# evanwporter/SparseCholesky

Measured on AMD Instinct MI355X. Metric: numeric-factorization fp64 GFLOP/s (F=sum colcount^2), higher is better.
Workload: dtype f64

## Files before the change

sparsecholesky_amd/csrc/kernels.hip:

```cpp
#include <hip/hip_runtime.h>

#include <cstdint>
#include <type_traits>

#include "kernels.hpp"

namespace sc {

typedef double double4_t __attribute__((ext_vector_type(4)));

__device__ __forceinline__ void report_fail(int32_t* info, const int32_t* post, int32_t col_internal) {
    atomicMin(info, (post ? post[col_internal] : col_internal) + 1);
}

__device__ __forceinline__ int bnd_at(const int32_t* b, int k, int mbc) {
    const int klo = b[0], khi = b[1];
    return k <= klo ? b[2] : (k >= khi ? mbc : b[2 + k - klo]);
}

__device__ __forceinline__ int lower_bound_i32(const int32_t* a, int n, int v) {
    int lo = 0, hi = n;
    while (lo < hi) {
        int mid = (lo + hi) >> 1;
        if (a[mid] < v)
// ... 839 lines not shown
            const double l = (ok && i > j) ? rec[j * 64 + i] / sqrt(d) : 0.0;
            lv[i] = l;
            wave_lds_sync();
            for (int k = j + 1; k < n; ++k)
                if (i >= k) rec[k * 64 + i] -= l * lv[k];
        }
    }
    if (i == 0) {
        if (T.host_info) {
            const int32_t st = fail < n ? nat + 1 : 0x7f7f7f7f;
            P.info[0] = st;
            __hip_atomic_store(T.host_info, st, __ATOMIC_RELEASE, __HIP_MEMORY_SCOPE_SYSTEM);
        } else if (fail < n) {
            atomicMin(P.info, nat + 1);
        }
    }
}

hipError_t launch_tiny_dense(const DevPlan& P, const TinyPlan& T, int n, const double* Ax, hipStream_t st) {
    if (n <= 0) return hipSuccess;
    if (n > TINY_DENSE_N || T.na != tiny_dense_np(n) * 64) return hipErrorInvalidValue;
    if ((int64_t)T.nax * 8 >= BUF_DEAD || (int64_t)T.npan * 8 >= BUF_DEAD) return hipErrorInvalidValue;
    if (n <= 16)
        hipLaunchKernelGGL(tiny_dense_kernel<16>, dim3(1), dim3(64), 0, st, P, T, n, Ax);
    else if (n <= 32)
        hipLaunchKernelGGL(tiny_dense_kernel<32>, dim3(1), dim3(64), 0, st, P, T, n, Ax);
    else if (n <= 48)
        hipLaunchKernelGGL(tiny_dense_kernel<48>, dim3(1), dim3(64), 0, st, P, T, n, Ax);
    else
        hipLaunchKernelGGL(tiny_dense_kernel<64>, dim3(1), dim3(64), 0, st, P, T, n, Ax);
    return hipGetLastError();
}

__global__ __launch_bounds__(256) void chain_init_kernel(DevPlan P, ChainPlan C, int first,
                                                          const double* __restrict__ Ax) {
    extern __shared__ double F[];
    const ChainDesc d = C.desc[first + blockIdx.x];
    small_assemble(P, d.s, d.c0, d.w, d.m, Ax, F, d.sp);
    const int tot = (d.m * (d.m + 1)) >> 1;
    double* out = C.init + d.init_off;
    for (int idx = threadIdx.x; idx < tot; idx += 256) out[idx] = F[idx];
}

#ifndef SC_CHAIN_DB
#define SC_CHAIN_DB 1
#endif
constexpr int CHAIN_IMG = (128 * 129 / 2 + CHAIN_NT - 1) / CHAIN_NT;
__global__ __launch_bounds__(CHAIN_NT) void front_chain_kernel(DevPlan P, ChainPlan C, int first, int count, int fsz) {
    extern __shared__ double F[];
    __shared__ __attribute__((aligned(16))) double colbuf[2 * 4 * COLB];
    __shared__ ChainDesc ds[CHAIN_MAXF];
    const int tid = threadIdx.x;
    for (int i = tid; i < count; i += CHAIN_NT) ds[i] = C.desc[first + i];
    lds_barrier();
    double img[CHAIN_IMG];
    int nbi, nbj;
    uint32_t nrr, nrc;
    auto prefetch = [&](int f) {
        const ChainDesc& d = ds[f];
        const int tot = (d.m * (d.m + 1)) >> 1;
        const double* src = C.init + d.init_off;
#pragma unroll
        for (int q = 0; q < CHAIN_IMG; ++q) {
            const int idx = tid + CHAIN_NT * q;
            img[q] = idx < tot ? src[idx] : 0.0;
        }
        const int T = (d.m + 3) >> 2;
        nbi = nbj = -1;
        if (tid < T * (T + 1) / 2) tile_map(tid, T, (d.w + 3) >> 2, nbi, nbj);
        nrr = nbi >= 0 ? C.relp[d.relp_off + nbi] : 0u;
        nrc = nbi >= 0 ? C.relp[d.relp_off + nbj] : 0u;
    };
    auto Fb = [&](int f) { return SC_CHAIN_DB ? F + (f & 1) * fsz : F; };
    auto put = [&](int f) {
        const int tot = (ds[f].m * (ds[f].m + 1)) >> 1;
        double* Fd = Fb(f);
#pragma unroll
        for (int q = 0; q < CHAIN_IMG; ++q) {
            const int idx = tid + CHAIN_NT * q;
            if (idx < tot) Fd[idx] = img[q];
        }
    };
    int cbi, cbj;
    uint32_t crr, crc;
    auto take = [&]() {
        cbi = nbi;
        cbj = nbj;
        crr = nrr;
        crc = nrc;
    };
    prefetch(0);
    put(0);
    take();
    if (count > 1) prefetch(1);
    lds_barrier();
    for (int i = 0; i < count; ++i) {
        uint64_t* stamp = C.stamps ? C.stamps + 8 * (first + i) : nullptr;
        if (stamp && tid == 0) stamp[0] = __builtin_amdgcn_s_memtime();
        const ChainDesc d = ds[i];
        const int m = d.m, w = d.w;
        SmallRegs<1> R;
        R.bi[0] = cbi;
        R.bj[0] = cbj;
        const uint32_t rr = crr, rc = crc;
        small_load<1>(R, Fb(i), m);
        if (!SC_CHAIN_DB) lds_barrier();
        if (stamp && tid == 0) stamp[1] = __builtin_amdgcn_s_memtime();
        const bool has_parent = i + 1 < count;
        if (has_parent) {
            put(i + 1);
            take();
            if (i + 2 < count) prefetch(i + 2);
        }
        if (stamp && tid == 0) stamp[2] = __builtin_amdgcn_s_memtime();
        small_steps<1>(R, colbuf, w, P.info, P.post, d.c0);
        if (w == 0) lds_barrier();
        if (stamp && tid == 0) stamp[3] = __builtin_amdgcn_s_memtime();
        small_store_panel<1>(R, P.panel_pool + d.panel_off, m, w);
        if (m > w && R.bi[0] >= 0 && 4 * R.bi[0] + 3 >= w) {
            if (!has_parent) {
                small_store_cb<1>(R, P.cb_pool + d.cb_off, m, w);
            } else {
                const int mp = ds[i + 1].m;
                double* Fp = Fb(i + 1);
#pragma unroll
                for (int r = 0; r < 4; ++r)
#pragma unroll
                    for (int c = 0; c < 4; ++c) {
                        const int ii = 4 * R.bi[0] + r, jj = 4 * R.bj[0] + c;
                        const int pr = (rr >> (8 * r)) & 255, pc = (rc >> (8 * c)) & 255;
                        if (jj >= w && ii >= jj && ii < m) Fp[pk_col(mp, pc) + pr - pc] += R.v[0][r * 4 + c];
                    }
            }
        }
        lds_barrier();
        if (stamp && tid == 0) stamp[4] = __builtin_amdgcn_s_memtime();
    }
}

#include "panel_gen.inc"

__global__ __launch_bounds__(256) void potrf_tiles_kernel(DevPlan P, const int2* __restrict__ tasks) {
    __shared__ __attribute__((aligned(16))) double colbuf[2 * 4 * COLB];
    const int2 t = tasks[blockIdx.x];
    const int s = t.x, k0 = t.y;
    const int c0 = P.sn_start[s];
    const int w = P.sn_start[s + 1] - c0;
    const int m = P.sn_m[s];
    const int nb = min(PNB, w - k0);
    double* blk = P.panel_pool + P.panel_off[s] + (int64_t)k0 * m + k0;
    SmallRegs<1> R;
    small_tiles<1>(R, nb, nb);
#pragma unroll
    for (int r = 0; r < 4; ++r)
#pragma unroll
        for (int c = 0; c < 4; ++c) {
            const int i = 4 * R.bi[0] + r, j = 4 * R.bj[0] + c;
            R.v[0][r * 4 + c] = (R.bi[0] >= 0 && i < nb && i >= j) ? blk[(int64_t)j * m + i] : 0.0;
        }
    if (SC_POTRF_FAST)
        small_steps1_fast(R, colbuf, nb, P.info, P.post, c0 + k0);
    else
        small_steps<1>(R, colbuf, nb, P.info, P.post, c0 + k0);
    if (R.bi[0] < 0) return;
#pragma unroll
    for (int r = 0; r < 4; ++r)
#pragma unroll
        for (int c = 0; c < 4; ++c) {
            const int i = 4 * R.bi[0] + r, j = 4 * R.bj[0] + c;
            if (i < nb && i >= j) blk[(int64_t)j * m + i] = R.v[0][r * 4 + c];
        }
}

__device__ __forceinline__ void trsm_partial(double* pan, int m, int k0, int nb, int r0, int nrows, double* Lc,
                                             double* invd) {
    constexpr int LD = PNB + 2;
    const int tid = threadIdx.x;
    const double* blk = pan + (int64_t)k0 * m + k0;
    for (int idx = tid; idx < PNB * PNB; idx += TRSM_ROWS) {
        const int q = idx % PNB, j = idx / PNB;
        const double v = (q < nb && j < nb && j <= q) ? blk[(int64_t)j * m + q] : 0.0;
        Lc[j * LD + q] = v;
        if (q == j) invd[j] = (j < nb) ? 1.0 / v : 0.0;
    }
    __syncthreads();
    const int row = r0 + tid;
    const bool live = row < m && tid < nrows;
    double* xs = pan + (int64_t)k0 * m + (live ? row : r0);
    double r[PNB];
#pragma unroll
    for (int c = 0; c < PNB; ++c) r[c] = (live && c < nb) ? xs[(int64_t)c * m] : 0.0;
    trsm_steps<0>(r, Lc, invd, nb);
    if (live) {
#pragma unroll
        for (int c = 0; c < PNB; ++c)
            if (c < nb) xs[(int64_t)c * m] = r[c];
    }
}

__global__ __launch_bounds__(TRSM_ROWS) void trsm_partial_kernel(DevPlan P, const TrsmTask* __restrict__ tasks) {
    __shared__ double Lc[PNB * (PNB + 2)];
    __shared__ double invd[PNB];
    const TrsmTask t = tasks[blockIdx.x];
    const int s = t.s, k0 = t.k0, r0 = t.r0;
    const int c0 = P.sn_start[s];
    const int w = P.sn_start[s + 1] - c0;
    const int m = P.sn_m[s];
    trsm_partial(P.panel_pool + P.panel_off[s], m, k0, min(PNB, w - k0), r0, min(TRSM_ROWS, t.r1 - r0), Lc, invd);
}

template <int PRE>
__global__ __launch_bounds__(TRSM_ROWS) void trsm_panel_g_kernel(DevPlan P, const TrsmTask* __restrict__ tasks,
                                                                 int32_t* __restrict__ arrive) {
    static_assert(TRSM_ROWS == 256, "the fused POTRF maps 4 x 4 tiles onto 256 threads");
    __shared__ double2 S[TRSM64_STREAM / 2];
    __shared__ __attribute__((aligned(16))) double colbuf[2 * 4 * COLB];
    __shared__ int s_last;
    const TrsmTask t = tasks[blockIdx.x];
    const int s = t.s, k0 = t.k0, r0 = t.r0, r1 = t.r1;
    const int tid = threadIdx.x;
    const int c0 = P.sn_start[s];
    const int w = P.sn_start[s + 1] - c0;
    const int m = P.sn_m[s];
    const int nb = min(PNB, w - k0);
    double* pan = P.panel_pool + P.panel_off[s];
    if (nb < PNB) return;
    double* blk = pan + (int64_t)k0 * m + k0;
    double* Sd = reinterpret_cast<double*>(S);
    SmallRegs<1> R;
    small_tiles<1>(R, PNB, PNB);
#pragma unroll
    for (int r = 0; r < 4; ++r)
#pragma unroll
        for (int c = 0; c < 4; ++c) {
            const int i = 4 * R.bi[0] + r, j = 4 * R.bj[0] + c;
            R.v[0][r * 4 + c] = (R.bi[0] >= 0 && i >= j) ? blk[(int64_t)j * m + i] : 0.0;
        }
    if constexpr (PRE == 2) {
        if (R.bi[0] >= 0) {
#pragma unroll
            for (int r = 0; r < 4; ++r)
#pragma unroll
                for (int c = 0; c < 4; ++c) {
                    const int i = 4 * R.bi[0] + r, j = 4 * R.bj[0] + c;
                    if (i >= j) Sd[PNB * j - j * (j - 1) / 2 + (i - j)] = (i == j) ? 1.0 / R.v[0][r * 4 + c] : R.v[0][r * 4 + c];
                }
        }
        const int row = r0 + tid;
        const __amdgpu_buffer_rsrc_t rs = buf_rsrc(pan + (int64_t)k0 * m, (uint32_t)m * PNB * 8u);
        const int voff = row < r1 ? row * 8 : BUF_DEAD;
        double r[PNB];
#pragma unroll
        for (int c = 0; c < PNB; ++c) r[c] = buf_ld(rs, voff, c * m * 8);
        __syncthreads();
        trsm64_full(r, S);
#pragma unroll
        for (int c = 0; c < PNB; ++c) buf_st(r[c], rs, voff, c * m * 8);
        return;
    }
    if (SC_POTRF_FAST)
        small_steps1_fast(R, colbuf, PNB, P.info, P.post, c0 + k0);
    else
        small_steps<1>(R, colbuf, PNB, P.info, P.post, c0 + k0);
    if (R.bi[0] >= 0) {
#pragma unroll
        for (int r = 0; r < 4; ++r)
#pragma unroll
            for (int c = 0; c < 4; ++c) {
                const int i = 4 * R.bi[0] + r, j = 4 * R.bj[0] + c;
                if (i >= j) Sd[PNB * j - j * (j - 1) / 2 + (i - j)] = (i == j) ? 1.0 / R.v[0][r * 4 + c] : R.v[0][r * 4 + c];
            }
    }
    const int row = r0 + tid;
    const __amdgpu_buffer_rsrc_t rs = buf_rsrc(pan + (int64_t)k0 * m, (uint32_t)m * PNB * 8u);
    const int voff = row < r1 ? row * 8 : BUF_DEAD;
    double r[PNB];
#pragma unroll
    for (int c = 0; c < PNB; ++c) r[c] = buf_ld(rs, voff, c * m * 8);
    __syncthreads();
    if (tid == 0) {
        const int k1 = k0 + PNB;
        const int nwg = (max(r1, k1 + 1) - k1 + TRSM_ROWS - 1) / TRSM_ROWS;
        const int old = __hip_atomic_fetch_add(arrive + (t.ctr - 1), 1, __ATOMIC_RELAXED, __HIP_MEMORY_SCOPE_AGENT);
        s_last = old == nwg - 1;
        if (old == nwg - 1) __hip_atomic_store(arrive + (t.ctr - 1), 0, __ATOMIC_RELAXED, __HIP_MEMORY_SCOPE_AGENT);
    }
    __syncthreads();
    if (s_last && R.bi[0] >= 0) {
#pragma unroll
        for (int rr = 0; rr < 4; ++rr)
#pragma unroll
            for (int c = 0; c < 4; ++c) {
                const int i = 4 * R.bi[0] + rr, j = 4 * R.bj[0] + c;
                if (i >= j) blk[(int64_t)j * m + i] = R.v[0][rr * 4 + c];
            }
    }
    trsm64_full(r, S);
#pragma unroll
    for (int c = 0; c < PNB; ++c) buf_st(r[c], rs, voff, c * m * 8);
}

#ifndef SC_PROBE_NOGATHER
#define SC_PROBE_NOGATHER 0
#endif
#ifndef SC_PROBE_NOK
#define SC_PROBE_NOK 0
#endif
template <int BT, int WM, int WN, int BK = 16, int GR = 64>
__device__ __forceinline__ void syrk_gather_epilogue(const GemmTask& T, const int64_t* __restrict__ gblk,
                                                     const GSeg* __restrict__ gseg, int row0, int col0,
                                                     double4_t (&acc)[BT / WM / 16][BT / WN / 16], double* smem) {
    constexpr int NW = WM * WN, NT = 64 * NW;
    constexpr int RTM = BT / WM / 16, RTN = BT / WN / 16;
    constexpr int GLD = GR + 1;
    constexpr int GQ = BT == 64 ? (GR == 32 ? 8 : 64 / NW) : SC_GATHER_Q;
    constexpr int SB = BT == 64 ? 4 : 1;
    constexpr int OPS = 2 * 2 * BK * (BT + 16);
    static_assert(BT * GLD <= OPS, "gather chunk fits the operand LDS");
    const int tid = threadIdx.x, lane = tid & 63, wid = tid >> 6;
    const int wr = wid / WN, wc = wid % WN;
    const int w = T.gw;
    const int mb = T.M;
    const int nb = (mb + 63) >> 6;
    const int64_t* __restrict__ blk = gblk + T.gb;
    const GSeg* __restrict__ seg = gseg;
    double* G = smem;
    double* __restrict__ C = T.C;
    const int64_t ldc = T.ldc;
    const __amdgpu_buffer_rsrc_t rc = buf_rsrc(C + (int64_t)col0 * ldc, (uint32_t)(min(BT, T.N - col0) * ldc * 8));
#pragma unroll 1
    for (int h = 0; h < BT / GR; ++h) {
        const int r0 = row0 + h * GR;
        const int rb = r0 >> 6;
        if (h) __syncthreads();
        for (int e = tid; e < BT * GLD; e += NT) G[e] = 0.0;
        __syncthreads();
        const int cb1 = min(min(nb, rb + 1), (col0 + BT) >> 6);
        for (int cbk = col0 >> 6; !SC_PROBE_NOGATHER && r0 < mb && cbk < cb1; ++cbk) {
            const int64_t bi = (int64_t)rb * (rb + 1) / 2 + cbk;
            const int64_t p0 = blk[bi], p1 = blk[bi + 1];
            for (int64_t pb = p0; pb < p1; pb += SB) {
                int prw[SB], pcl[SB];
#pragma unroll
                for (int q = 0; q < SB; ++q) {
                    prw[q] = -1;
                    pcl[q] = -1;
                    if (pb + q < p1) {
                        const GSeg& g = seg[pb + q];
                        const int ic = g.ilo + lane, jl = g.jlo + lane;
                        if (ic < g.ihi) prw[q] = g.rel[ic] - w - r0;
                        if (jl < g.jhi) pcl[q] = g.rel[jl] - w - col0;
                    }
                }
#pragma unroll
                for (int q = 0; q < SB; ++q) {
                    if (pb + q >= p1) break;
                    const GSeg& g = seg[pb + q];
                    const int ic = g.ilo + lane;
                    const int prow = prw[q] < GR ? prw[q] : -1;
                    const int mbc = g.mbc;
                    const double* __restrict__ cb = g.cb;
                    uint64_t mask = __ballot(pcl[q] >= 0 && pcl[q] % NW == wid);
                    while (mask) {
                        int jc[GQ], pc[GQ];
#pragma unroll
                        for (int u = 0; u < GQ; ++u) {
                            const int b = mask ? __builtin_ctzll(mask) : -1;
                            jc[u] = b < 0 ? -1 : g.jlo + b;
                            pc[u] = b < 0 ? 0 : __builtin_amdgcn_readlane(pcl[q], b);
                            mask &= mask - 1;
                        }
                        double v[GQ];
                        bool ok[GQ];
#pragma unroll
                        for (int u = 0; u < GQ; ++u) {
                            ok[u] = jc[u] >= 0 && prow >= 0 && ic >= jc[u];
                            const __amdgpu_buffer_rsrc_t rs = buf_rsrc(cb + (int64_t)max(jc[u], 0) * mbc, (uint32_t)mbc * 8u);
                            v[u] = buf_ld(rs, ok[u] ? ic * 8 : BUF_DEAD, 0);
                        }
#pragma unroll
                        for (int u = 0; u < GQ; ++u)
                            if (ok[u]) G[pc[u] * GLD + prow] += v[u];
                    }
                }
            }
        }
        __syncthreads();
        static_assert(GR % (BT / WM) == 0, "a wave's rows lie in one chunk");
        if ((wr * (BT / WM)) / GR == h) {
#pragma unroll
            for (int a = 0; a < RTM; ++a)
#pragma unroll
                for (int b = 0; b < RTN; ++b)
#pragma unroll
                    for (int r = 0; r < 4; ++r) {
                        const int lr = wr * (BT / WM) + a * 16 + MFMA_F64_ROW(lane, r);
                        const int lc = wc * (BT / WN) + b * 16 + (lane & 15);
                        G[lc * GLD + (lr - h * GR)] -= acc[a][b][r];
                    }
        }
        __syncthreads();
#pragma unroll 4
        for (int e = tid; e < BT * GR; e += NT) {
            const int lr = e % GR, lc = e / GR;
            const int gi = r0 + lr, gj = col0 + lc;
            const bool live = gi < T.M && gi >= gj && gj < T.N;
            buf_st(G[lc * GLD + lr], rc, live ? (int)((gi + (int64_t)(gj - col0) * ldc) * 8) : BUF_DEAD, 0);
        }
    }
}

template <int BT, int WM, int WN, int BK = 16, int GR = 64>
__device__ __forceinline__ void syrk_rmw_epilogue(const GemmTask& T, int row0, int col0,
                                                  double4_t (&acc)[BT / WM / 16][BT / WN / 16], double* smem) {
    constexpr int NW = WM * WN, NT = 64 * NW;
    constexpr int RTM = BT / WM / 16, RTN = BT / WN / 16;
    constexpr int GLD = GR + 1;
    constexpr int OPS = 2 * 2 * BK * (BT + 16);
    static_assert(BT * GLD <= OPS, "chunk fits the operand LDS");
    static_assert(GR % (BT / WM) == 0, "a wave's rows lie in one chunk");
    const int tid = threadIdx.x, lane = tid & 63, wid = tid >> 6;
    const int wr = wid / WN, wc = wid % WN;
    double* G = smem;
    const int64_t ldc = T.ldc;
    const __amdgpu_buffer_rsrc_t rc = buf_rsrc(T.C + (int64_t)col0 * ldc, (uint32_t)(min(BT, T.N - col0) * ldc * 8));
#pragma unroll 1
    for (int h = 0; h < BT / GR; ++h) {
        const int r0 = row0 + h * GR;
        if (h) __syncthreads();
#pragma unroll 4
        for (int e = tid; e < BT * GR; e += NT) {
            const int lr = e % GR, lc = e / GR;
            const int gi = r0 + lr, gj = col0 + lc;
            const bool live = gi < T.M && gi >= gj && gj < T.N;
            G[lc * GLD + lr] = buf_ld(rc, live ? (int)((gi + (int64_t)(gj - col0) * ldc) * 8) : BUF_DEAD, 0);
        }
        __syncthreads();
        if ((wr * (BT / WM)) / GR == h) {
#pragma unroll
            for (int a = 0; a < RTM; ++a)
#pragma unroll
                for (int b = 0; b < RTN; ++b)
#pragma unroll
                    for (int r = 0; r < 4; ++r) {
                        const int lr = wr * (BT / WM) + a * 16 + MFMA_F64_ROW(lane, r);
                        const int lc = wc * (BT / WN) + b * 16 + (lane & 15);
                        G[lc * GLD + (lr - h * GR)] -= acc[a][b][r];
                    }
        }
        __syncthreads();
#pragma unroll 4
        for (int e = tid; e < BT * GR; e += NT) {
            const int lr = e % GR, lc = e / GR;
            const int gi = r0 + lr, gj = col0 + lc;
            const bool live = gi < T.M && gi >= gj && gj < T.N;
            buf_st(G[lc * GLD + lr], rc, live ? (int)((gi + (int64_t)(gj - col0) * ldc) * 8) : BUF_DEAD, 0);
        }
    }
}

template <int BT, int WM, int WN, int BK = 16>
__device__ __forceinline__ void mfma_kloop(const double* __restrict__ A, int64_t lda, int K, int M, int N, int row0,
                                           int col0, double4_t (&acc)[BT / WM / 16][BT / WN / 16], double* smem) {
    static_assert(BK == 16 || BK == 8, "four-deep k sub-steps of the MFMA");
    constexpr int NT = 64 * WM * WN;
    constexpr int LDT = BT + 16;
    constexpr int RTM = BT / WM / 16, RTN = BT / WN / 16;
    double(*As)[BK * LDT] = reinterpret_cast<double(*)[BK * LDT]>(smem);
    double(*Bs)[BK * LDT] = reinterpret_cast<double(*)[BK * LDT]>(smem + 2 * BK * LDT);
    const int tid = threadIdx.x;
    const int lane = tid & 63;
    const int wid = tid >> 6;
    const int wr = wid / WN, wc = wid % WN;
    constexpr int PER = BT * BK / NT;
    double ra[PER], rb[PER];
    auto gload = [&](int k0) {
        const __amdgpu_buffer_rsrc_t rs = buf_rsrc(A + (int64_t)k0 * lda, (uint32_t)(min(BK, K - k0) * lda * 8));
#pragma unroll
        for (int q = 0; q < PER; ++q) {
            const int e = tid + q * NT;
            const int r = e % BT, kk = e / BT;
            const int gr = row0 + r, gc = col0 + r;
            ra[q] = buf_ld(rs, gr < M ? (int)((gr + kk * lda) * 8) : BUF_DEAD, 0);
            rb[q] = buf_ld(rs, gc < N ? (int)((gc + kk * lda) * 8) : BUF_DEAD, 0);
        }
    };
    auto sstore = [&](int buf) {
#pragma unroll
        for (int q = 0; q < PER; ++q) {
            const int e = tid + q * NT;
            const int r = e % BT, kk = e / BT;
            As[buf][kk * LDT + r] = ra[q];
            Bs[buf][kk * LDT + r] = rb[q];
        }
    };

    const int nk = (K + BK - 1) / BK;
    auto stage = [&](int kt, auto last) {
        constexpr bool LAST = decltype(last)::value;
        const int cur = kt & 1;
        if (!LAST) gload((kt + 1) * BK);
        double av[2][RTM], bv[2][RTN];
        auto lread = [&](int kk, int slot) {
            const int krow = kk + (lane >> 4);
#pragma unroll
            for (int a = 0; a < RTM; ++a)
                av[slot][a] = As[cur][krow * LDT + wr * (BT / WM) + a * 16 + (lane & 15)];
#pragma unroll
            for (int b = 0; b < RTN; ++b)
                bv[slot][b] = Bs[cur][krow * LDT + wc * (BT / WN) + b * 16 + (lane & 15)];
        };
        lread(0, 0);
#pragma unroll
        for (int kk = 0; kk < BK; kk += 4) {
            const int slot = (kk / 4) & 1;
            if (kk + 4 < BK) lread(kk + 4, slot ^ 1);
#pragma unroll
            for (int a = 0; a < RTM; ++a)
#pragma unroll
                for (int b = 0; b < RTN; ++b)
                    acc[a][b] = __builtin_amdgcn_mfma_f64_16x16x4f64(av[slot][a], bv[slot][b], acc[a][b], 0, 0, 0);
            if (!LAST && kk == BK - 8) sstore(cur ^ 1);
        }
        __syncthreads();
    };
    gload(0);
    sstore(0);
    __syncthreads();
    for (int kt = 0; kt + 1 < nk; ++kt) stage(kt, std::false_type {});
    if (nk > 0) stage(nk - 1, std::true_type {});
}

template <int BK>
__device__ __forceinline__ void panel_prefactor(const GemmTask& T, int32_t* info, const int32_t* post,
                                                double* smem) {
    static_assert(2 * 2 * BK * (64 + 16) >= 64 * 65 / 2, "the packed diagonal block fits the operand LDS");
    double4_t acc[2][2];
#pragma unroll
    for (int a = 0; a < 2; ++a)
#pragma unroll
        for (int b = 0; b < 2; ++b) acc[a][b] = (double4_t){0.0, 0.0, 0.0, 0.0};
    mfma_kloop<64, 2, 2, BK>(T.A, T.lda, T.K, T.M, T.N, 0, 0, acc, smem);
    const int tid = threadIdx.x, lane = tid & 63, wid = tid >> 6;
    const int wr = wid >> 1, wc = wid & 1;
    const int64_t ldc = T.ldc;
    double* __restrict__ F = smem;
    const __amdgpu_buffer_rsrc_t rc = buf_rsrc(T.C, (uint32_t)(64 * ldc * 8));
    double cv[2][2][4];
#pragma unroll
    for (int a = 0; a < 2; ++a)
#pragma unroll
        for (int b = 0; b < 2; ++b)
#pragma unroll
            for (int r = 0; r < 4; ++r) {
                const int gi = wr * 32 + a * 16 + MFMA_F64_ROW(lane, r), gj = wc * 32 + b * 16 + (lane & 15);
                cv[a][b][r] = buf_ld(rc, gi >= gj ? (int)((gi + (int64_t)gj * ldc) * 8) : BUF_DEAD, 0);
            }
#pragma unroll
    for (int a = 0; a < 2; ++a)
#pragma unroll
        for (int b = 0; b < 2; ++b)
#pragma unroll
            for (int r = 0; r < 4; ++r) {
                const int gi = wr * 32 + a * 16 + MFMA_F64_ROW(lane, r), gj = wc * 32 + b * 16 + (lane & 15);
                if (gi >= gj) F[pk_col(64, gj) + gi - gj] = cv[a][b][r] - acc[a][b][r];
            }
    __syncthreads();
    SmallRegs<1> R;
    small_tiles<1>(R, PNB, PNB);
    small_load<1>(R, F, PNB);
    __syncthreads();
    small_steps1_fast(R, smem, PNB, info, post, T.pf);
    if (R.bi[0] < 0) return;
#pragma unroll
    for (int r = 0; r < 4; ++r)
#pragma unroll
        for (int c = 0; c < 4; ++c) {
            const int i = 4 * R.bi[0] + r, j = 4 * R.bj[0] + c;
            if (i >= j) T.C[(int64_t)j * ldc + i] = R.v[0][r * 4 + c];
        }
}

template <int BT, int WM, int WN, int TAG, int EPI, int LEAN = 0, int PF = 0>
__device__ __forceinline__ void syrk_tile_body(const GemmTask* __restrict__ tasks, const int2* __restrict__ tiles,
                                               int bidx, const int64_t* __restrict__ gblk,
                                               const GSeg* __restrict__ gseg, int32_t* info = nullptr,
                                               const int32_t* post = nullptr) {
    constexpr int BK = LEAN ? 8 : 16;
    constexpr int LDT = BT + 16;
    constexpr int RTM = BT / WM / 16, RTN = BT / WN / 16;
    __shared__ __attribute__((aligned(16))) double smem[2 * 2 * BK * LDT];

    const int2 tl = tiles[bidx];
    const GemmTask T = tasks[tl.x];
    if constexpr (PF) {
        static_assert(BT == 64 && WM == 2 && WN == 2 && TAG == 0, "pre-factor on 64 x 64 panel-update tiles");
        if (tl.y < 0) {
            panel_prefactor<BK>(T, info, post, smem);
            return;
        }
    }
    const int ti = tl.y >> 16, tj = tl.y & 0xffff;
    const int row0 = ti * BT, col0 = tj * BT;

    const int wid = threadIdx.x >> 6;
    if (wid >= WM * WN / 2) __builtin_amdgcn_s_setprio(1);

    double4_t acc[RTM][RTN];
#pragma unroll
    for (int a = 0; a < RTM; ++a)
#pragma unroll
        for (int b = 0; b < RTN; ++b) acc[a][b] = (double4_t){0.0, 0.0, 0.0, 0.0};
    if (!(SC_PROBE_NOK && TAG == 1 && T.gs >= 0)) mfma_kloop<BT, WM, WN, BK>(T.A, T.lda, T.K, T.M, T.N, row0, col0, acc, smem);

    if constexpr (TAG == 1) {
        if (T.gs >= 0) {
            syrk_gather_epilogue<BT, WM, WN, BK, LEAN ? 32 : 64>(T, gblk, gseg, row0, col0, acc, smem);
            return;
        }
    }
    syrk_rmw_epilogue<BT, WM, WN, BK, LEAN ? 32 : 64>(T, row0, col0, acc, smem);
}

template <int BT, int WM, int WN, int TAG, int EPI, int LEAN = 0, int PF = 0>
__global__ __launch_bounds__(64 * WM * WN, LEAN ? (TAG ? 5 : 6) : 1) void syrk_mfma_kernel(const GemmTask* __restrict__ tasks,
                                                                  const int2* __restrict__ tiles,
                                                                  const int64_t* __restrict__ gblk,
                                                                  const GSeg* __restrict__ gseg, int32_t* info,
                                                                  const int32_t* post) {
    syrk_tile_body<BT, WM, WN, TAG, EPI, LEAN, PF>(tasks, tiles, blockIdx.x, gblk, gseg, info, post);
}

static int small_kt(int maxm) {
    const int T = (maxm + 3) / 4;
    return (T * (T + 1) / 2 + 255) / 256;
}

hipError_t launch_front_small(const DevPlan& P, const int32_t* nodes, int count, int maxm, bool seq,
                              const double* Ax, hipStream_t st) {
    if (count <= 0) return hipSuccess;
    const size_t lds = (size_t)maxm * (maxm + 1) / 2 * sizeof(double);
    const int kt = small_kt(maxm);
    const dim3 grid(seq ? 1 : count);
    const int sq = seq ? count : 0;
    if (kt <= 1)
        hipLaunchKernelGGL(front_small_kernel<1>, grid, dim3(256), lds, st, P, nodes, Ax, sq);
    else if (kt == 2)
        hipLaunchKernelGGL(front_small_kernel<2>, grid, dim3(256), lds, st, P, nodes, Ax, sq);
    else
        hipLaunchKernelGGL(front_small_kernel<3>, grid, dim3(256), lds, st, P, nodes, Ax, sq);
    return hipGetLastError();
}

hipError_t launch_front_chain(const DevPlan& P, const ChainPlan& C, int first, int count, int maxm,
                              const double* Ax, hipStream_t st) {
    if (count <= 0) return hipSuccess;
    if (count > CHAIN_MAXF || maxm > 128) return hipErrorInvalidValue;
    const int fsz = maxm * (maxm + 1) / 2;
    const size_t lds = (size_t)fsz * sizeof(double);
    hipLaunchKernelGGL(chain_init_kernel, dim3(count), dim3(256), lds, st, P, C, first, Ax);
    hipLaunchKernelGGL(front_chain_kernel, dim3(1), dim3(CHAIN_NT), (SC_CHAIN_DB ? 2 : 1) * lds, st, P, C, first, count,
                       fsz);
    return hipGetLastError();
}

hipError_t launch_assemble_large(const DevPlan& P, const int2* tasks, int count, const double* Ax,
                                 hipStream_t st, bool tiled, const int2* lim) {
    if (count <= 0) return hipSuccess;
    if (tiled)
        hipLaunchKernelGGL(assemble_tile_kernel, dim3(count), dim3(256), 0, st, P, tasks, Ax, lim);
    else
        hipLaunchKernelGGL(assemble_cols_kernel, dim3(count), dim3(256), 0, st, P, tasks, Ax);
    return hipGetLastError();
}

hipError_t launch_potrf_diag(const DevPlan& P, const int2* tasks, int count, hipStream_t st) {
    if (count <= 0) return hipSuccess;
    hipLaunchKernelGGL(potrf_tiles_kernel, dim3(count), dim3(256), 0, st, P, tasks);
    return hipGetLastError();
}

hipError_t launch_trsm_panel(const DevPlan& P, const TrsmTask* tasks, int count, hipStream_t st, bool partial,
                             int32_t* arrive, int pre) {
    if (count <= 0) return hipSuccess;
    if (partial)
        hipLaunchKernelGGL(trsm_partial_kernel, dim3(count), dim3(TRSM_ROWS), 0, st, P, tasks);
    else if (pre == 2)
        hipLaunchKernelGGL(trsm_panel_g_kernel<2>, dim3(count), dim3(TRSM_ROWS), 0, st, P, tasks, arrive);
    else
        hipLaunchKernelGGL(trsm_panel_g_kernel<0>, dim3(count), dim3(TRSM_ROWS), 0, st, P, tasks, arrive);
    return hipGetLastError();
}

template <int TAG, int EPI>
static void launch_syrk_t(const GemmTask* tasks, const int2* tiles, int n, int bt, hipStream_t st, GatherTab gt,
                          bool lean) {
    if (bt == 64 && lean)
        hipLaunchKernelGGL((syrk_mfma_kernel<64, 2, 2, TAG, EPI, 1>), dim3(n), dim3(256), 0, st, tasks, tiles, gt.blk,
                           gt.seg, gt.info, gt.post);
    else if (bt == 128)
        hipLaunchKernelGGL((syrk_mfma_kernel<128, 2, 4, TAG, EPI>), dim3(n), dim3(512), 0, st, tasks, tiles, gt.blk,
                           gt.seg, gt.info, gt.post);
    else
        hipLaunchKernelGGL((syrk_mfma_kernel<64, 2, 2, TAG, EPI>), dim3(n), dim3(256), 0, st, tasks, tiles, gt.blk,
                           gt.seg, gt.info, gt.post);
}

hipError_t launch_syrk(const GemmTask* tasks, const int2* tiles, int total_tiles, int bt, int tag, hipStream_t st,
                       int epi, GatherTab gt, bool lean, bool pf) {
    if (total_tiles <= 0) return hipSuccess;
    if (pf) {
        if (bt != 64 || tag) return hipErrorInvalidValue;
        hipLaunchKernelGGL((syrk_mfma_kernel<64, 2, 2, 0, 1, 0, 1>), dim3(total_tiles), dim3(256), 0, st, tasks, tiles,
                           gt.blk, gt.seg, gt.info, gt.post);
        return hipGetLastError();
    }
    if (tag)
        epi ? launch_syrk_t<1, 1>(tasks, tiles, total_tiles, bt, st, gt, lean)
            : launch_syrk_t<1, 0>(tasks, tiles, total_tiles, bt, st, gt, lean);
    else
        epi ? launch_syrk_t<0, 1>(tasks, tiles, total_tiles, bt, st, gt, lean)
            : launch_syrk_t<0, 0>(tasks, tiles, total_tiles, bt, st, gt, lean);
    return hipGetLastError();
}

__global__ void fill_random_kernel(double* p, int64_t n) {
    for (int64_t i = blockIdx.x * (int64_t)blockDim.x + threadIdx.x; i < n; i += (int64_t)gridDim.x * blockDim.x) {
        uint64_t x = (uint64_t)i * 0x9E3779B97F4A7C15ull;
        x ^= x >> 31;
        x *= 0xBF58476D1CE4E5B9ull;
        x ^= x >> 29;
        p[i] = (double)(x >> 11) * (2.0 / 9007199254740992.0) - 1.0;
    }
}

hipError_t launch_fill_random(double* p, int64_t n, hipStream_t st) {
    hipLaunchKernelGGL(fill_random_kernel, dim3(1024), dim3(256), 0, st, p, n);
    return hipGetLastError();
}

__global__ void stamp_kernel(uint64_t* slot) { *slot = __builtin_amdgcn_s_memrealtime(); }

__global__ void status_publish_kernel(int32_t* info, int32_t* host) {
    const int32_t v = __hip_atomic_load(info, __ATOMIC_RELAXED, __HIP_MEMORY_SCOPE_AGENT);
    __hip_atomic_store(info, 0x7f7f7f7f, __ATOMIC_RELAXED, __HIP_MEMORY_SCOPE_AGENT);
    __hip_atomic_store(host, v, __ATOMIC_RELEASE, __HIP_MEMORY_SCOPE_SYSTEM);
}

hipError_t launch_status_publish(int32_t* info, int32_t* host, hipStream_t st) {
    hipLaunchKernelGGL(status_publish_kernel, dim3(1), dim3(1), 0, st, info, host);
    return hipGetLastError();
}

__global__ void hwid_kernel(uint32_t* out, int spin) {
    if (threadIdx.x == 0) {
        out[2 * blockIdx.x] = __builtin_amdgcn_s_getreg((31 << 11) | 4);
        out[2 * blockIdx.x + 1] = __builtin_amdgcn_s_getreg((15 << 11) | 20);
    }
    const uint64_t t0 = __builtin_amdgcn_s_memrealtime();
    while (__builtin_amdgcn_s_memrealtime() - t0 < (uint64_t)spin) __builtin_amdgcn_s_sleep(8);
}

hipError_t launch_hwid(uint32_t* out, int nwg, int threads, int spin, hipStream_t st) {
    hipLaunchKernelGGL(hwid_kernel, dim3(nwg), dim3(threads), 0, st, out, spin);
    return hipGetLastError();
}

hipError_t launch_stamp(uint64_t* slot, hipStream_t st) {
    hipLaunchKernelGGL(stamp_kernel, dim3(1), dim3(1), 0, st, slot);
    return hipGetLastError();
}

__global__ __launch_bounds__(256) void copy2d_kernel(const Copy2D* __restrict__ descs, const int2* __restrict__ tiles,
                                                     int unpack) {
    const int2 t = tiles[blockIdx.x];
    const Copy2D d = descs[t.x];
    const int lane = threadIdx.x & 63, wid = threadIdx.x >> 6;
    const int j0 = t.y & 0xffff, r0 = (t.y >> 16) * COPY_ROWS;
    const int j1 = min(d.cols, j0 + COPY_COLS), r1 = min(d.rows, r0 + COPY_ROWS);
    for (int j = j0 + wid; j < j1; j += 4) {
        const double* __restrict__ src = unpack ? d.b + (int64_t)j * d.rows : d.a + (int64_t)j * d.lda;
        double* __restrict__ dst = unpack ? d.a + (int64_t)j * d.lda : d.b + (int64_t)j * d.rows;
        for (int r = r0 + lane; r < r1; r += 64 * 8) {
            double v[8];
#pragma unroll
            for (int u = 0; u < 8; ++u) v[u] = r + 64 * u < r1 ? src[r + 64 * u] : 0.0;
#pragma unroll
            for (int u = 0; u < 8; ++u)
                if (r + 64 * u < r1) dst[r + 64 * u] = v[u];
        }
    }
}

hipError_t launch_copy2d(const Copy2D* descs, const int2* tiles, int count, bool unpack, hipStream_t st) {
    if (count <= 0) return hipSuccess;
    hipLaunchKernelGGL(copy2d_kernel, dim3(count), dim3(256), 0, st, descs, tiles, unpack ? 1 : 0);
    return hipGetLastError();
}

template <int NACC>
__global__ __launch_bounds__(256) void mfma_peak_kernel(double* out, int iters) {
    double4_t acc[NACC];
#pragma unroll
    for (int j = 0; j < NACC; ++j) acc[j] = (double4_t){0.0, 0.0, 0.0, 0.0};
    const double a = 1.0 + threadIdx.x * 1e-9, b = 1.0 - blockIdx.x * 1e-9;
    for (int i = 0; i < iters; i += 16) {
#pragma unroll
        for (int u = 0; u < 16; ++u)
#pragma unroll
            for (int j = 0; j < NACC; ++j) acc[j] = __builtin_amdgcn_mfma_f64_16x16x4f64(a, b, acc[j], 0, 0, 0);
    }
    double s = 0.0;
#pragma unroll
    for (int j = 0; j < NACC; ++j) s += acc[j][0] + acc[j][1] + acc[j][2] + acc[j][3];
    if (s == 1234.5) out[blockIdx.x] = s;
}

hipError_t launch_mfma_peak(double* out, int blocks, int iters, int nacc, hipStream_t st) {
    if (nacc == 16)
        hipLaunchKernelGGL((mfma_peak_kernel<16>), dim3(blocks), dim3(256), 0, st, out, iters);
    else if (nacc == 8)
        hipLaunchKernelGGL((mfma_peak_kernel<8>), dim3(blocks), dim3(256), 0, st, out, iters);
    else if (nacc == 2)
        hipLaunchKernelGGL((mfma_peak_kernel<2>), dim3(blocks), dim3(256), 0, st, out, iters);
    else
        hipLaunchKernelGGL((mfma_peak_kernel<4>), dim3(blocks), dim3(256), 0, st, out, iters);
    return hipGetLastError();
}

__global__ __launch_bounds__(64) void solve_inv_kernel(SolvePlan P, const int2* __restrict__ tasks) {
    __shared__ double2 S[TRSM64_STREAM / 2];
    __shared__ double Lc[PNB * (PNB + 2)];
    __shared__ double invd[PNB];
    const int2 t = tasks[blockIdx.x];
    const int s = t.x, k0 = t.y;
    const int lane = threadIdx.x;
    const int c0 = P.sn_start[s];
    const int w = P.sn_start[s + 1] - c0;
    const int m = P.sn_m[s];
    const int nb = min(PNB, w - k0);
    double* blk = const_cast<double*>(P.panel_pool) + P.panel_off[s] + (int64_t)k0 * m + k0;
    double r[PNB];
    {
#pragma unroll
        for (int j = 0; j < PNB; ++j) r[j] = (j < nb && lane < nb && lane >= j) ? blk[(int64_t)j * m + lane] : 0.0;
    }
    if (nb == PNB) {
        double* Sd = reinterpret_cast<double*>(S);
#pragma unroll
        for (int j = 0; j < PNB; ++j)
            if (lane >= j) Sd[PNB * j - j * (j - 1) / 2 + (lane - j)] = lane == j ? 1.0 / r[j] : r[j];
    } else {
        constexpr int LD = PNB + 2;
#pragma unroll
        for (int j = 0; j < PNB; ++j) {
            Lc[j * LD + lane] = r[j];
            if (lane == j) invd[j] = j < nb ? 1.0 / r[j] : 0.0;
        }
    }
    __syncthreads();
#pragma unroll
    for (int c = 0; c < PNB; ++c) r[c] = c == lane ? 1.0 : 0.0;
    if (nb == PNB)
        trsm64_full(r, S);
    else
        trsm_steps<0>(r, Lc, invd, nb);
#pragma unroll
    for (int c = 0; c < PNB; ++c)
        if (lane < c && c < nb) blk[(int64_t)c * m + lane] = r[c];
}

__global__ __launch_bounds__(256) void solve_inv2_kernel(SolvePlan P, const int2* __restrict__ tasks) {
    __shared__ double Xa[PNB][PNB + 1], Bm[PNB][PNB + 1], Xb[PNB][PNB + 1];
    const int2 t = tasks[blockIdx.x];
    const int s = t.x, k0 = t.y;
    const int tid = threadIdx.x;
    const int c0 = P.sn_start[s];
    const int w = P.sn_start[s + 1] - c0;
    const int m = P.sn_m[s];
    const int nbb = min(SOLVE_NB, w - k0) - PNB;
    double* blk = const_cast<double*>(P.panel_pool) + P.panel_off[s] + (int64_t)k0 * m + k0;
    const double* blkb = blk + (int64_t)PNB * m + PNB;
#pragma unroll
    for (int q = 0; q < PNB * PNB / 256; ++q) {
        const int e = tid + 256 * q, i = e >> 6, k = e & 63;
        Xa[i][k] = k < i ? blk[(int64_t)i * m + k] : (k == i ? 1.0 / blk[(int64_t)i * m + i] : 0.0);
        Xb[i][k] = (i < nbb && k < i) ? blkb[(int64_t)i * m + k] : ((i < nbb && k == i) ? 1.0 / blkb[(int64_t)i * m + i] : 0.0);
        Bm[k][i] = k < nbb ? blk[(int64_t)i * m + PNB + k] : 0.0;
    }
    __syncthreads();
    const int i = tid >> 2, jg = tid & 3;
    double acc[16];
#pragma unroll
    for (int q = 0; q < 16; ++q) acc[q] = 0.0;
    for (int k = 0; k < PNB; ++k) {
        const double bik = Bm[i][k];
#pragma unroll
        for (int q = 0; q < 16; ++q) acc[q] = fma(bik, Xa[k][jg + 4 * q], acc[q]);
    }
    __syncthreads();
#pragma unroll
    for (int q = 0; q < 16; ++q) Bm[i][jg + 4 * q] = acc[q];
    __syncthreads();
#pragma unroll
    for (int q = 0; q < 16; ++q) acc[q] = 0.0;
    for (int k = 0; k <= i; ++k) {
        const double xik = Xb[i][k];
#pragma unroll
        for (int q = 0; q < 16; ++q) acc[q] = fma(xik, Bm[k][jg + 4 * q], acc[q]);
    }
    if (i < nbb) {
#pragma unroll
        for (int q = 0; q < 16; ++q) blk[(int64_t)(PNB + i) * m + jg + 4 * q] = -acc[q];
    }
}

__device__ __forceinline__ void quad_apply(const double* __restrict__ blk, int64_t m, int nb, int I, int K,
                                           const double* cb, double* out, bool add, double (*part)[PNB],
                                           double (*Xs)[PNB + 1]) {
    const int tid = threadIdx.x;
    const __amdgpu_buffer_rsrc_t rs = buf_rsrc(blk, (uint32_t)(((int64_t)(nb - 1) * m + nb) * 8));
    double v[PNB * PNB / 256];
#pragma unroll
    for (int q = 0; q < PNB * PNB / 256; ++q) {
        const int e = tid + 256 * q, i = e >> 6, k = e & 63;
        const int gi = PNB * I + i, gk = PNB * K + k;
        v[q] = buf_ld(rs, (gi < nb && gk <= gi) ? (int)(((int64_t)gi * m + gk) * 8) : BUF_DEAD, 0);
    }
// ... 1113 lines not shown
```

Baseline: 57980.

## Deepen k-loop prefetch ring and preload C during prologue for prefactor kernels

For the pre-factor (PF) SYRK kernel, the MFMA k-loop now keeps a ring of PD register sets (default 2), so global loads run several k-steps ahead. The C-tile read for the read-modify-write epilogue (and for the diagonal pre-factor) is issued right after the prologue loads, so its latency overlaps the k-loop instead of sitting in the epilogue. Launch bounds ask for 3 waves per SIMD occupancy on these variants. This costs extra registers per thread for the prefetch sets and the preloaded C values, which could cause spills or lower occupancy.

Result: no change. 58210, median of 6 (+0.4%).

```diff
diff --git a/sparsecholesky_amd/csrc/kernels.hip b/sparsecholesky_amd/csrc/kernels.hip
--- a/sparsecholesky_amd/csrc/kernels.hip
+++ b/sparsecholesky_amd/csrc/kernels.hip
@@ -1165,6 +1165,12 @@
 
 #ifndef SC_PROBE_NOGATHER
 #define SC_PROBE_NOGATHER 0
+#endif
+#ifndef SC_KLOOP_PD
+#define SC_KLOOP_PD 2
+#endif
+#ifndef SC_SHORTK_CPRE
+#define SC_SHORTK_CPRE 1
 #endif
 #ifndef SC_PROBE_NOK
 #define SC_PROBE_NOK 0
@@ -1273,15 +1279,33 @@
     }
 }
 
-template <int BT, int WM, int WN, int BK = 16, int GR = 64>
+template <int BT, int NT>
+__device__ __forceinline__ void rmw_c_preload(const GemmTask& T, int row0, int col0, double (&c)[BT * BT / NT]) {
+    static_assert(NT % BT == 0, "a thread keeps its row: entry e = tid + q NT is (tid % BT, tid / BT + q NT / BT)");
+    const int tid = threadIdx.x;
+    const int64_t ldc = T.ldc;
+    const __amdgpu_buffer_rsrc_t rc = buf_rsrc(T.C + (int64_t)col0 * ldc, (uint32_t)(min(BT, T.N - col0) * ldc * 8));
+    const int gi = row0 + tid % BT, lc0 = tid / BT;
+#pragma unroll
+    for (int q = 0; q < BT * BT / NT; ++q) {
+        const int lc = lc0 + q * (NT / BT);
+        const int gj = col0 + lc;
+        const bool live = gi < T.M && gi >= gj && gj < T.N;
+        c[q] = buf_ld(rc, live ? (int)((gi + (int64_t)lc * ldc) * 8) : BUF_DEAD, 0);
+    }
+}
+
+template <int BT, int WM, int WN, int BK = 16, int GR = 64, bool CPRE = false>
 __device__ __forceinline__ void syrk_rmw_epilogue(const GemmTask& T, int row0, int col0,
-                                                  double4_t (&acc)[BT / WM / 16][BT / WN / 16], double* smem) {
+                                                  double4_t (&acc)[BT / WM / 16][BT / WN / 16], double* smem,
+                                                  const double* cpre = nullptr) {
     constexpr int NW = WM * WN, NT = 64 * NW;
     constexpr int RTM = BT / WM / 16, RTN = BT / WN / 16;
     constexpr int GLD = GR + 1;
     constexpr int OPS = 2 * 2 * BK * (BT + 16);
     static_assert(BT * GLD <= OPS, "chunk fits the operand LDS");
     static_assert(GR % (BT / WM) == 0, "a wave's rows lie in one chunk");
+    static_assert(!CPRE || BT == GR, "preloaded C: the tile is one chunk");
     const int tid = threadIdx.x, lane = tid & 63, wid = tid >> 6;
     const int wr = wid / WN, wc = wid % WN;
     double* G = smem;
@@ -1291,12 +1315,18 @@
     for (int h = 0; h < BT / GR; ++h) {
         const int r0 = row0 + h * GR;
         if (h) __syncthreads();
+        if constexpr (CPRE) {
+            double* Gt = G + (tid / GR) * GLD + tid % GR;
+#pragma unroll
+            for (int q = 0; q < BT * GR / NT; ++q) Gt[q * (NT / GR) * GLD] = cpre[q];
+        } else {
 #pragma unroll 4
-        for (int e = tid; e < BT * GR; e += NT) {
-            const int lr = e % GR, lc = e / GR;
-            const int gi = r0 + lr, gj = col0 + lc;
-            const bool live = gi < T.M && gi >= gj && gj < T.N;
-            G[lc * GLD + lr] = buf_ld(rc, live ? (int)((gi + (int64_t)(gj - col0) * ldc) * 8) : BUF_DEAD, 0);
+            for (int e = tid; e < BT * GR; e += NT) {
+                const int lr = e % GR, lc = e / GR;
+                const int gi = r0 + lr, gj = col0 + lc;
+                const bool live = gi < T.M && gi >= gj && gj < T.N;
+                G[lc * GLD + lr] = buf_ld(rc, live ? (int)((gi + (int64_t)(gj - col0) * ldc) * 8) : BUF_DEAD, 0);
+            }
         }
         __syncthreads();
         if ((wr * (BT / WM)) / GR == h) {
@@ -1322,10 +1352,15 @@
     }
 }
 
-template <int BT, int WM, int WN, int BK = 16>
+struct KloopNop {
+    __device__ __forceinline__ void operator()() const {}
+};
+template <int BT, int WM, int WN, int BK = 16, int PD = 1, class AfterPrologue = KloopNop>
 __device__ __forceinline__ void mfma_kloop(const double* __restrict__ A, int64_t lda, int K, int M, int N, int row0,
-                                           int col0, double4_t (&acc)[BT / WM / 16][BT / WN / 16], double* smem) {
+                                           int col0, double4_t (&acc)[BT / WM / 16][BT / WN / 16], double* smem,
+                                           AfterPrologue after_prologue = AfterPrologue()) {
     static_assert(BK == 16 || BK == 8, "four-deep k sub-steps of the MFMA");
+    static_assert(PD >= 1 && PD <= 4, "register sets of the prefetch ring");
     constexpr int NT = 64 * WM * WN;
     constexpr int LDT = BT + 16;
     constexpr int RTM = BT / WM / 16, RTN = BT / WN / 16;
@@ -1336,33 +1371,34 @@
     const int wid = tid >> 6;
     const int wr = wid / WN, wc = wid % WN;
     constexpr int PER = BT * BK / NT;
-    double ra[PER], rb[PER];
-    auto gload = [&](int k0) {
-        const __amdgpu_buffer_rsrc_t rs = buf_rsrc(A + (int64_t)k0 * lda, (uint32_t)(min(BK, K - k0) * lda * 8));
+    double ra[PD][PER], rb[PD][PER];
+    auto gload = [&](int k0, int set) {
+        const int ncol = PD == 1 ? min(BK, K - k0) : __builtin_amdgcn_readfirstlane(max(0, min(BK, K - k0)));
+        const __amdgpu_buffer_rsrc_t rs = buf_rsrc(A + (int64_t)k0 * lda, (uint32_t)(ncol * lda * 8));
 #pragma unroll
         for (int q = 0; q < PER; ++q) {
             const int e = tid + q * NT;
             const int r = e % BT, kk = e / BT;
             const int gr = row0 + r, gc = col0 + r;
-            ra[q] = buf_ld(rs, gr < M ? (int)((gr + kk * lda) * 8) : BUF_DEAD, 0);
-            rb[q] = buf_ld(rs, gc < N ? (int)((gc + kk * lda) * 8) : BUF_DEAD, 0);
+            ra[set][q] = buf_ld(rs, gr < M ? (int)((gr + kk * lda) * 8) : BUF_DEAD, 0);
+            rb[set][q] = buf_ld(rs, gc < N ? (int)((gc + kk * lda) * 8) : BUF_DEAD, 0);
         }
     };
-    auto sstore = [&](int buf) {
+    auto sstore = [&](int buf, int set) {
 #pragma unroll
         for (int q = 0; q < PER; ++q) {
             const int e = tid + q * NT;
             const int r = e % BT, kk = e / BT;
-            As[buf][kk * LDT + r] = ra[q];
-            Bs[buf][kk * LDT + r] = rb[q];
+            As[buf][kk * LDT + r] = ra[set][q];
+            Bs[buf][kk * LDT + r] = rb[set][q];
         }
     };
 
     const int nk = (K + BK - 1) / BK;
-    auto stage = [&](int kt, auto last) {
+    auto stage = [&](int kt, int set, auto last) {
         constexpr bool LAST = decltype(last)::value;
         const int cur = kt & 1;
-        if (!LAST) gload((kt + 1) * BK);
+        if (!LAST) gload((kt + PD) * BK, set);
         double av[2][RTM], bv[2][RTN];
         auto lread = [&](int kk, int slot) {
             const int krow = kk + (lane >> 4);
@@ -1383,18 +1419,42 @@
 #pragma unroll
                 for (int b = 0; b < RTN; ++b)
                     acc[a][b] = __builtin_amdgcn_mfma_f64_16x16x4f64(av[slot][a], bv[slot][b], acc[a][b], 0, 0, 0);
-            if (!LAST && kk == BK - 8) sstore(cur ^ 1);
+            if (!LAST && kk == BK - 8) sstore(cur ^ 1, (set + 1) % PD);
         }
         __syncthreads();
     };
-    gload(0);
-    sstore(0);
+    gload(0, 0);
+    if constexpr (PD > 1) {
+#pragma unroll
+        for (int s = 1; s < PD; ++s) gload(s * BK, s);
+    }
+    if constexpr (!std::is_same<AfterPrologue, KloopNop>::value) after_prologue();
+    sstore(0, 0);
     __syncthreads();
-    for (int kt = 0; kt + 1 < nk; ++kt) stage(kt, std::false_type {});
-    if (nk > 0) stage(nk - 1, std::true_type {});
-}
-
-template <int BK>
+    if constexpr (PD == 1) {
+        for (int kt = 0; kt + 1 < nk; ++kt) stage(kt, 0, std::false_type {});
+        if (nk > 0) stage(nk - 1, 0, std::true_type {});
+    } else {
+        int kt = 0;
+        for (; kt + PD < nk; kt += PD)
+#pragma unroll
+            for (int s = 0; s < PD; ++s) stage(kt + s, s, std::false_type {});
+        auto close = [&](auto self, auto jc) {
+            constexpr int J = decltype(jc)::value;
+            if constexpr (J + 1 < PD) {
+                if (kt + J + 1 < nk) {
+                    stage(kt + J, J, std::false_type {});
+                    self(self, std::integral_constant<int, J + 1> {});
+                    return;
+                }
+            }
+            stage(kt + J, J, std::true_type {});
+        };
+        if (nk > 0) close(close, std::integral_constant<int, 0> {});
+    }
+}
+
+template <int BK, int PD = 1, bool CPRE = false>
 __device__ __forceinline__ void panel_prefactor(const GemmTask& T, int32_t* info, const int32_t* post,
                                                 double* smem) {
     static_assert(2 * 2 * BK * (64 + 16) >= 64 * 65 / 2, "the packed diagonal block fits the operand LDS");
@@ -1403,22 +1463,29 @@
     for (int a = 0; a < 2; ++a)
 #pragma unroll
         for (int b = 0; b < 2; ++b) acc[a][b] = (double4_t){0.0, 0.0, 0.0, 0.0};
-    mfma_kloop<64, 2, 2, BK>(T.A, T.lda, T.K, T.M, T.N, 0, 0, acc, smem);
     const int tid = threadIdx.x, lane = tid & 63, wid = tid >> 6;
     const int wr = wid >> 1, wc = wid & 1;
     const int64_t ldc = T.ldc;
     double* __restrict__ F = smem;
     const __amdgpu_buffer_rsrc_t rc = buf_rsrc(T.C, (uint32_t)(64 * ldc * 8));
     double cv[2][2][4];
-#pragma unroll
-    for (int a = 0; a < 2; ++a)
-#pragma unroll
-        for (int b = 0; b < 2; ++b)
-#pragma unroll
-            for (int r = 0; r < 4; ++r) {
-                const int gi = wr * 32 + a * 16 + MFMA_F64_ROW(lane, r), gj = wc * 32 + b * 16 + (lane & 15);
-                cv[a][b][r] = buf_ld(rc, gi >= gj ? (int)((gi + (int64_t)gj * ldc) * 8) : BUF_DEAD, 0);
-            }
+    auto cload = [&]() {
+#pragma unroll
+        for (int a = 0; a < 2; ++a)
+#pragma unroll
+            for (int b = 0; b < 2; ++b)
+#pragma unroll
+                for (int r = 0; r < 4; ++r) {
+                    const int gi = wr * 32 + a * 16 + MFMA_F64_ROW(lane, r), gj = wc * 32 + b * 16 + (lane & 15);
+                    cv[a][b][r] = buf_ld(rc, gi >= gj ? (int)((gi + (int64_t)gj * ldc) * 8) : BUF_DEAD, 0);
+                }
+    };
+    if constexpr (CPRE) {
+        mfma_kloop<64, 2, 2, BK, PD>(T.A, T.lda, T.K, T.M, T.N, 0, 0, acc, smem, cload);
+    } else {
+        mfma_kloop<64, 2, 2, BK, PD>(T.A, T.lda, T.K, T.M, T.N, 0, 0, acc, smem);
+        cload();
+    }
 #pragma unroll
     for (int a = 0; a < 2; ++a)
 #pragma unroll
@@ -1452,6 +1519,8 @@
     constexpr int BK = LEAN ? 8 : 16;
     constexpr int LDT = BT + 16;
     constexpr int RTM = BT / WM / 16, RTN = BT / WN / 16;
+    constexpr int PD = PF ? SC_KLOOP_PD : 1;
+    constexpr bool CPRE = PF && SC_SHORTK_CPRE;
     __shared__ __attribute__((aligned(16))) double smem[2 * 2 * BK * LDT];
 
     const int2 tl = tiles[bidx];
@@ -1459,7 +1528,7 @@
     if constexpr (PF) {
         static_assert(BT == 64 && WM == 2 && WN == 2 && TAG == 0, "pre-factor on 64 x 64 panel-update tiles");
         if (tl.y < 0) {
-            panel_prefactor<BK>(T, info, post, smem);
+            panel_prefactor<BK, PD, CPRE>(T, info, post, smem);
             return;
         }
     }
@@ -1474,7 +1543,14 @@
     for (int a = 0; a < RTM; ++a)
 #pragma unroll
         for (int b = 0; b < RTN; ++b) acc[a][b] = (double4_t){0.0, 0.0, 0.0, 0.0};
-    if (!(SC_PROBE_NOK && TAG == 1 && T.gs >= 0)) mfma_kloop<BT, WM, WN, BK>(T.A, T.lda, T.K, T.M, T.N, row0, col0, acc, smem);
+    if constexpr (CPRE) {
+        double cpre[BT * BT / (64 * WM * WN)];
+        mfma_kloop<BT, WM, WN, BK, PD>(T.A, T.lda, T.K, T.M, T.N, row0, col0, acc, smem,
+                                       [&]() { rmw_c_preload<BT, 64 * WM * WN>(T, row0, col0, cpre); });
+        syrk_rmw_epilogue<BT, WM, WN, BK, 64, true>(T, row0, col0, acc, smem, cpre);
+        return;
+    }
+    if (!(SC_PROBE_NOK && TAG == 1 && T.gs >= 0)) mfma_kloop<BT, WM, WN, BK, PD>(T.A, T.lda, T.K, T.M, T.N, row0, col0, acc, smem);
 
     if constexpr (TAG == 1) {
         if (T.gs >= 0) {
@@ -1486,7 +1562,7 @@
 }
 
 template <int BT, int WM, int WN, int TAG, int EPI, int LEAN = 0, int PF = 0>
-__global__ __launch_bounds__(64 * WM * WN, LEAN ? (TAG ? 5 : 6) : 1) void syrk_mfma_kernel(const GemmTask* __restrict__ tasks,
+__global__ __launch_bounds__(64 * WM * WN, LEAN ? (TAG ? 5 : 6) : (PF && (SC_KLOOP_PD > 1 || SC_SHORTK_CPRE)) ? 3 : 1) void syrk_mfma_kernel(const GemmTask* __restrict__ tasks,
                                                                   const int2* __restrict__ tiles,
                                                                   const int64_t* __restrict__ gblk,
                                                                   const GSeg* __restrict__ gseg, int32_t* info,
```
